# GiorgiaAuroraAdorni/gansformer-reproducibility-challenge

Measured on NVIDIA H100. Metric: images/sec @256^2 synth (GANsformer generator forward, K=16 latents, 12 attention layers, batch 32/GPU), higher is better.
Workload: dtype tf32 (fp32 storage; wgmma tf32 attention and stride-1 3x3 convolutions (own kernels), TF32 cuDNN up-convolutions; value_fp32_convs = the same with fp32 cuDNN convolutions)

## Files before the change

### gansformer-reproducibility-challenge_b200/csrc/gf_conv.cu

```cuda
#include <stdlib.h>
#include <string.h>
#include "gf_common.cuh"
#include "gf_tc_common.cuh"
#include "../../include/gf_ops.h"

namespace gf {
namespace cv {

using namespace tc;

constexpr int PH = 8, PW = 16;
constexpr int BK = 32;
constexpr int A_ROWS = (PH + 2) * PW;
constexpr int A_BYTES = A_ROWS * BK * 4;
constexpr int NUM_THREADS = 288;
constexpr int MAX_A = 3, MAX_W = 8;

struct Bars {
  uint64_t full_a[MAX_A], empty_a[MAX_A], full_w[MAX_W], empty_w[MAX_W];
};

struct Params {
  int B, H, W, Cin, Cout;
  int tiles_h, tiles_w, tiles_n;
  long long total_tiles;
  int na, nw;
  float alpha;
};

__device__ __forceinline__ void tma_load_4d(uint32_t dst, const CUtensorMap* map, uint32_t bar, int c0, int c1, int c2, int c3) {
  asm volatile(
      "cp.async.bulk.tensor.4d.shared::cluster.global.mbarrier::complete_tx::bytes [%0], [%1, {%3, %4, %5, %6}], [%2];"
      ::"r"(dst), "l"(map), "r"(bar), "r"(c0), "r"(c1), "r"(c2), "r"(c3)
      : "memory");
}

template <int BN>
__global__ void __launch_bounds__(NUM_THREADS, 1)
conv3x3_tc_kernel(const __grid_constant__ CUtensorMap tmX, const __grid_constant__ CUtensorMap tmW, float* __restrict__ y, const Params P) {
  constexpr int W_BYTES = BN * BK * 4;
  extern __shared__ __align__(1024) uint8_t smem_raw[];
  uint8_t* smem = smem_raw + ((1024u - (smem_u32(smem_raw) & 1023u)) & 1023u);
  const uint32_t s_a = smem_u32(smem);
  const uint32_t s_w = s_a + (uint32_t)P.na * A_BYTES;
  Bars* bars = reinterpret_cast<Bars*>(smem + (size_t)P.na * A_BYTES + (size_t)P.nw * W_BYTES);
  const int warp = __shfl_sync(0xffffffffu, (int)(threadIdx.x >> 5), 0);
  const int lane = threadIdx.x & 31;

  if (warp == 8 && lane == 0) {
    prefetch_tmap(&tmX); prefetch_tmap(&tmW);
    for (int i = 0; i < P.na; ++i) { mbar_init(smem_u32(&bars->full_a[i]), 1); mbar_init(smem_u32(&bars->empty_a[i]), 2); }
    for (int i = 0; i < P.nw; ++i) { mbar_init(smem_u32(&bars->full_w[i]), 1); mbar_init(smem_u32(&bars->empty_w[i]), 2); }
    fence_barrier_init();
  }
  __syncthreads();

  auto decode = [&](long long t, int& nt, int& pw, int& ph, int& b) {
    nt = (int)(t % P.tiles_n); t /= P.tiles_n;
    pw = (int)(t % P.tiles_w); t /= P.tiles_w;
    ph = (int)(t % P.tiles_h); b = (int)(t / P.tiles_h);
  };

  if (warp == 8) {
    if (lane == 0) {
      int sa = 0, sw = 0; uint32_t pa = 0, pw_ = 0;
      for (long long t = blockIdx.x; t < P.total_tiles; t += gridDim.x) {
        int nt, pw, ph, b;
        decode(t, nt, pw, ph, b);
        const int h0 = ph * PH, w0 = pw * PW, n0 = nt * BN;
        for (int c0 = 0; c0 < P.Cin; c0 += BK) {
          for (int dx = 0; dx < 3; ++dx) {
            mbar_wait(smem_u32(&bars->empty_a[sa]), pa ^ 1u);
            const uint32_t fa = smem_u32(&bars->full_a[sa]);
            mbar_expect_tx(fa, (uint32_t)A_BYTES);
            tma_load_4d(s_a + (uint32_t)sa * A_BYTES, &tmX, fa, c0, w0 + dx - 1, h0 - 1, b);
            if (++sa == P.na) { sa = 0; pa ^= 1u; }
            for (int dy = 0; dy < 3; ++dy) {
              mbar_wait(smem_u32(&bars->empty_w[sw]), pw_ ^ 1u);
              const uint32_t fw = smem_u32(&bars->full_w[sw]);
              mbar_expect_tx(fw, (uint32_t)W_BYTES);
              tma_load_2d(s_w + (uint32_t)sw * W_BYTES, &tmW, fw, c0, (dy * 3 + dx) * P.Cout + n0);
              if (++sw == P.nw) { sw = 0; pw_ ^= 1u; }
            }
          }
        }
      }
    }
    return;
  }

  const int wg = warp >> 2;
  const int gid = lane >> 2, qd = lane & 3;
  const int rA = wg * 64 + (warp & 3) * 16 + gid;
  const bool leader = (warp & 3) == 0 && lane == 0;
  int sa = 0, sw = 0; uint32_t pa = 0, pw_ = 0;
  for (long long t = blockIdx.x; t < P.total_tiles; t += gridDim.x) {
    int nt, pw, ph, b;
    decode(t, nt, pw, ph, b);
    float acc[BN / 2];
    int prev_w = -1, prev_a = -1;
#pragma unroll 1
    for (int c0 = 0; c0 < P.Cin; c0 += BK) {
#pragma unroll 1
      for (int dx = 0; dx < 3; ++dx) {
        mbar_wait(smem_u32(&bars->full_a[sa]), pa);
        const uint32_t a_view = s_a + (uint32_t)sa * A_BYTES + wg * 64 * 128;
#pragma unroll
        for (int dy = 0; dy < 3; ++dy) {
          mbar_wait(smem_u32(&bars->full_w[sw]), pw_);
          const uint64_t da = gmma_desc(a_view + dy * PW * 128, 1024, LAYOUT_SW128);
          const uint64_t db = gmma_desc(s_w + (uint32_t)sw * W_BYTES, 1024, LAYOUT_SW128);
          const uint32_t acc0 = (c0 | dx | dy) ? 1u : 0u;
          wgmma_fence();
#pragma unroll
          for (int kk = 0; kk < 4; ++kk) wgmma_ss<BN>(acc, da + kk * 2, db + kk * 2, (acc0 | kk) ? 1u : 0u);
          wgmma_commit();
          wgmma_wait<1>();
          if (prev_w >= 0) {
            named_bar_sync(1 + wg, 128);
            if (leader) {
              mbar_arrive(smem_u32(&bars->empty_w[prev_w]));
              if (prev_a >= 0) mbar_arrive(smem_u32(&bars->empty_a[prev_a]));
            }
          }
          prev_w = sw;
          prev_a = dy == 2 ? sa : -1;
          if (++sw == P.nw) { sw = 0; pw_ ^= 1u; }
        }
        if (++sa == P.na) { sa = 0; pa ^= 1u; }
      }
    }
    wgmma_wait<0>();
    fence_regs<BN / 2>(acc);
    named_bar_sync(1 + wg, 128);
    if (leader) {
      mbar_arrive(smem_u32(&bars->empty_w[prev_w]));
      mbar_arrive(smem_u32(&bars->empty_a[prev_a]));
    }
#pragma unroll
    for (int i = 0; i < 2; ++i) {
      const int r = rA + 8 * i;
      const int h = ph * PH + (r >> 4), w = pw * PW + (r & 15);
      float* yrow = y + (((size_t)b * P.H + h) * P.W + w) * P.Cout + nt * BN + 2 * qd;
#pragma unroll
      for (int j = 0; j < BN / 8; ++j)
        *reinterpret_cast<float2*>(yrow + 8 * j) = make_float2(acc[4 * j + 2 * i] * P.alpha, acc[4 * j + 2 * i + 1] * P.alpha);
    }
  }
}

constexpr int U_PC = 16, U_PR = 8;
constexpr int U_OC = U_PC - 2;
constexpr int U_BN = 64;
constexpr int U_A_BYTES = (U_PR + 1) * U_PC * BK * 4;
constexpr int U_W_BYTES = U_BN * BK * 4;
constexpr int U_CS = 68;
constexpr int U_MAX_A = 4, U_MAX_W = 10;

struct UBars {
  uint64_t full_a[U_MAX_A], empty_a[U_MAX_A], full_w[U_MAX_W], empty_w[U_MAX_W];
};

struct UParams {
  int B, H, W, Cin, Cout;
  int strips, steps, tiles_n;
  int total_units;
  int na, nw;
  float ag;
  const float* scale;
};

__device__ constexpr int U_TAP[9] = {0, 6, 3, 2, 1, 8, 7, 5, 4};
__device__ constexpr int U_PH[9] = {0, 0, 2, 0, 1, 0, 1, 2, 3};
__device__ constexpr int U_ROW0[9] = {1, 0, 0, 1, 1, 0, 0, 0, 0};
__device__ constexpr int U_FIRST[9] = {1, 0, 1, 0, 1, 0, 0, 0, 1};

__global__ void __launch_bounds__(NUM_THREADS, 1)
upconv_blur_tc_kernel(const __grid_constant__ CUtensorMap tmX, const __grid_constant__ CUtensorMap tmW, float* __restrict__ y, const UParams P) {
  extern __shared__ __align__(1024) uint8_t smem_raw[];
  uint8_t* smem = smem_raw + ((1024u - (smem_u32(smem_raw) & 1023u)) & 1023u);
  const uint32_t s_a = smem_u32(smem);
  const uint32_t s_w = s_a + (uint32_t)P.na * U_A_BYTES;
  float* carry = reinterpret_cast<float*>(smem + (size_t)P.na * U_A_BYTES + (size_t)P.nw * U_W_BYTES);
  float* stage = carry + 4 * 2 * U_PC * U_CS;
  UBars* bars = reinterpret_cast<UBars*>(stage + U_PR * U_PC * U_CS);
  const int warp = __shfl_sync(0xffffffffu, (int)(threadIdx.x >> 5), 0);
  const int lane = threadIdx.x & 31;

  if (warp == 8 && lane == 0) {
    prefetch_tmap(&tmX); prefetch_tmap(&tmW);
    for (int i = 0; i < P.na; ++i) { mbar_init(smem_u32(&bars->full_a[i]), 1); mbar_init(smem_u32(&bars->empty_a[i]), 2); }
    for (int i = 0; i < P.nw; ++i) { mbar_init(smem_u32(&bars->full_w[i]), 1); mbar_init(smem_u32(&bars->empty_w[i]), 2); }
    fence_barrier_init();
  }
  __syncthreads();

  auto decode = [&](int u, int& nt, int& st, int& b) {
    nt = u % P.tiles_n; u /= P.tiles_n;
    st = u % P.strips; b = u / P.strips;
  };

  if (warp == 8) {
    if (lane == 0) {
      int sa = 0, sw = 0; uint32_t pa = 0, pw_ = 0;
      for (int u = blockIdx.x; u < P.total_units; u += gridDim.x) {
        int nt, st, b;
        decode(u, nt, st, b);
        const int j0 = st * U_OC, n0 = nt * U_BN;
        for (int s = 0; s < P.steps; ++s) {
          for (int c0 = 0; c0 < P.Cin; c0 += BK) {
            for (int t = 0; t < 9; ++t) {
              if (t == 0 || t == 3) {
                mbar_wait(smem_u32(&bars->empty_a[sa]), pa ^ 1u);
                const uint32_t fa = smem_u32(&bars->full_a[sa]);
                mbar_expect_tx(fa, (uint32_t)U_A_BYTES);
                tma_load_4d(s_a + (uint32_t)sa * U_A_BYTES, &tmX, fa, c0, j0 - (t == 3), s * U_PR - 1, b);
                if (++sa == P.na) { sa = 0; pa ^= 1u; }
              }
              mbar_wait(smem_u32(&bars->empty_w[sw]), pw_ ^ 1u);
              const uint32_t fw = smem_u32(&bars->full_w[sw]);
              mbar_expect_tx(fw, (uint32_t)U_W_BYTES);
              tma_load_2d(s_w + (uint32_t)sw * U_W_BYTES, &tmW, fw, c0, U_TAP[t] * P.Cout + n0);
              if (++sw == P.nw) { sw = 0; pw_ ^= 1u; }
            }
          }
        }
      }
    }
    return;
  }

  const int wg = warp >> 2;
  const int gid = lane >> 2, qd = lane & 3;
  const bool leader = (warp & 3) == 0 && lane == 0;
  const int cp = lane & 7, cg = lane >> 3;
  int sa = 0, sw = 0; uint32_t pa = 0, pw_ = 0;
  for (int u = blockIdx.x; u < P.total_units; u += gridDim.x) {
    int nt, st, b;
    decode(u, nt, st, b);
    const int j0 = st * U_OC, n0 = nt * U_BN;
    for (int s = 0; s < P.steps; ++s) {
      float acc[4][U_BN / 2];
      int prev_w = -1, prev_a = -1;
      uint32_t a_view = 0;
#pragma unroll 1
      for (int c0 = 0; c0 < P.Cin; c0 += BK) {
#pragma unroll
        for (int t = 0; t < 9; ++t) {
          if (t == 0 || t == 3) {
            mbar_wait(smem_u32(&bars->full_a[sa]), pa);
            a_view = s_a + (uint32_t)sa * U_A_BYTES + wg * 4 * U_PC * 128;
          }
          mbar_wait(smem_u32(&bars->full_w[sw]), pw_);
          const uint64_t da = gmma_desc(a_view + U_ROW0[t] * U_PC * 128, 1024, LAYOUT_SW128);
          const uint64_t db = gmma_desc(s_w + (uint32_t)sw * U_W_BYTES, 1024, LAYOUT_SW128);
          const uint32_t acc0 = (c0 > 0 || !U_FIRST[t]) ? 1u : 0u;
          wgmma_fence();
#pragma unroll
          for (int kk = 0; kk < 4; ++kk) wgmma_ss<U_BN>(acc[U_PH[t]], da + kk * 2, db + kk * 2, (acc0 | kk) ? 1u : 0u);
          wgmma_commit();
          wgmma_wait<1>();
          if (prev_w >= 0) {
            named_bar_sync(1 + wg, 128);
            if (leader) {
              mbar_arrive(smem_u32(&bars->empty_w[prev_w]));
              if (prev_a >= 0) mbar_arrive(smem_u32(&bars->empty_a[prev_a]));
            }
          }
          prev_w = sw;
          prev_a = (t == 2 || t == 8) ? sa : -1;
          if (++sw == P.nw) { sw = 0; pw_ ^= 1u; }
          if (t == 2 || t == 8) { if (++sa == P.na) { sa = 0; pa ^= 1u; } }
        }
      }
      wgmma_wait<0>();
#pragma unroll
      for (int ph = 0; ph < 4; ++ph) fence_regs<U_BN / 2>(acc[ph]);
      named_bar_sync(1 + wg, 128);
      if (leader) {
        mbar_arrive(smem_u32(&bars->empty_w[prev_w]));
        mbar_arrive(smem_u32(&bars->empty_a[prev_a]));
      }

      const int io = s * U_PR - 2 + warp;
#pragma unroll
      for (int sl = 0; sl < U_BN / 16; ++sl) {
        float* my_row = stage + warp * U_PC * U_CS;
#pragma unroll
        for (int ph = 0; ph < 4; ++ph)
#pragma unroll
          for (int jj = 0; jj < 2; ++jj)
#pragma unroll
            for (int i = 0; i < 2; ++i)
              *reinterpret_cast<float2*>(my_row + (gid + 8 * i) * U_CS + ph * 16 + jj * 8 + 2 * qd) =
                  make_float2(acc[ph][4 * (2 * sl + jj) + 2 * i], acc[ph][4 * (2 * sl + jj) + 2 * i + 1]);
        named_bar_sync(3, 256);
        if (io >= 0 && io < P.H) {
          auto row = [&](int r) -> const float* {
            return (r < 2 ? carry + (sl * 2 + r) * U_PC * U_CS : stage + (r - 2) * U_PC * U_CS) + 2 * cp;
          };
          const int ch = n0 + sl * 16 + 2 * cp;
          const float2 d = __ldg(reinterpret_cast<const float2*>(P.scale + (size_t)b * P.Cout + ch));
          const float2 f = make_float2(P.ag * d.x, P.ag * d.y);
          const int Wo = 2 * P.W;
#pragma unroll 1
          for (int p = cg; p < U_OC && j0 + p < P.W; p += 4) {
            float* y0 = y + (((size_t)b * 2 * P.H + 2 * io) * Wo + 2 * (j0 + p)) * P.Cout + ch;
#pragma unroll 1
            for (int cb = 0; cb < 2; ++cb) {
              const int oA = cb ? 0 : 16, oB = cb ? U_CS + 16 : 0, oC = cb ? U_CS : U_CS + 16, oD = cb ? 2 * U_CS + 16 : U_CS;
              float2 e, o;
#pragma unroll
              for (int v = 0; v < 5; ++v) {
                const float* base = row(warp + v / 2) + ((v & 1) ? 0 : 32) + p * U_CS;
                const float2 A = *reinterpret_cast<const float2*>(base + oA), B_ = *reinterpret_cast<const float2*>(base + oB);
                const float2 C = *reinterpret_cast<const float2*>(base + oC), D = *reinterpret_cast<const float2*>(base + oD);
                float2 hv;
                hv.x = ((A.x + 3.f * B_.x) + 3.f * C.x) + D.x;
                hv.y = ((A.y + 3.f * B_.y) + 3.f * C.y) + D.y;
                if (v == 0) { e = hv; }
                else if (v == 1) { e.x += 3.f * hv.x; e.y += 3.f * hv.y; o = hv; }
                else if (v == 2) { e.x += 3.f * hv.x; e.y += 3.f * hv.y; o.x += 3.f * hv.x; o.y += 3.f * hv.y; }
                else if (v == 3) { e.x += hv.x; e.y += hv.y; o.x += 3.f * hv.x; o.y += 3.f * hv.y; }
                else { o.x += hv.x; o.y += hv.y; }
              }
              *reinterpret_cast<float2*>(y0 + cb * P.Cout) = make_float2(e.x * 0.015625f * f.x, e.y * 0.015625f * f.y);
              *reinterpret_cast<float2*>(y0 + (size_t)Wo * P.Cout + cb * P.Cout) = make_float2(o.x * 0.015625f * f.x, o.y * 0.015625f * f.y);
            }
          }
        }
        named_bar_sync(3, 256);
        if (warp >= U_PR - 2) {
          float* crow = carry + (sl * 2 + warp - (U_PR - 2)) * U_PC * U_CS;
#pragma unroll
          for (int ph = 0; ph < 4; ++ph)
#pragma unroll
            for (int jj = 0; jj < 2; ++jj)
#pragma unroll
              for (int i = 0; i < 2; ++i)
                *reinterpret_cast<float2*>(crow + (gid + 8 * i) * U_CS + ph * 16 + jj * 8 + 2 * qd) =
                    make_float2(acc[ph][4 * (2 * sl + jj) + 2 * i], acc[ph][4 * (2 * sl + jj) + 2 * i + 1]);
        }
      }
    }
  }
}

static int make_map_nhwc(CUtensorMap* m, const void* base, int B, int H, int W, int C, int box_c, int box_w, int box_h) {
  EncodeTiledFn enc = get_encode();
  if (!enc) { set_error("cuTensorMapEncodeTiled entry point not available"); return GF_ERR_CUDA; }
  cuuint64_t dims[4] = {(cuuint64_t)C, (cuuint64_t)W, (cuuint64_t)H, (cuuint64_t)B};
  cuuint64_t strides[3] = {(cuuint64_t)C * 4, (cuuint64_t)W * C * 4, (cuuint64_t)H * W * C * 4};
  cuuint32_t box[4] = {(cuuint32_t)box_c, (cuuint32_t)box_w, (cuuint32_t)box_h, 1};
  cuuint32_t estr[4] = {1, 1, 1, 1};
  CUresult r = enc(m, CU_TENSOR_MAP_DATA_TYPE_FLOAT32, 4, const_cast<void*>(base), dims, strides, box, estr, CU_TENSOR_MAP_INTERLEAVE_NONE,
                   CU_TENSOR_MAP_SWIZZLE_128B, CU_TENSOR_MAP_L2_PROMOTION_L2_128B, CU_TENSOR_MAP_FLOAT_OOB_FILL_NONE);
  if (r != CUDA_SUCCESS) { set_error("cuTensorMapEncodeTiled (NHWC 4-D) failed with CUresult %d (B=%d H=%d W=%d C=%d)", (int)r, B, H, W, C); return GF_ERR_CUDA; }
  return GF_OK;
}

template <int BN>
static int launch_bn(const float* x, const float* wt, float* y, int B, int H, int W, int Cin, int Cout, cudaStream_t st) {
  constexpr int W_BYTES = BN * BK * 4;
  CUtensorMap tmX, tmW;
  int rc;
  if ((rc = make_map_nhwc(&tmX, x, B, H, W, Cin, BK, PW, PH + 2))) return rc;
  if ((rc = make_map(&tmW, wt, (uint64_t)9 * Cout, (uint64_t)Cin, BN, BK, CU_TENSOR_MAP_SWIZZLE_128B))) return rc;
  Params P;
  P.B = B; P.H = H; P.W = W; P.Cin = Cin; P.Cout = Cout;
  P.tiles_h = H / PH; P.tiles_w = W / PW; P.tiles_n = Cout / BN;
  P.total_tiles = (long long)B * P.tiles_h * P.tiles_w * P.tiles_n;
  const int avail = device_smem_optin() - (int)sizeof(Bars) - 1024;
  P.na = MAX_A;
  P.nw = (avail - P.na * A_BYTES) / W_BYTES;
  if (P.nw > MAX_W) P.nw = MAX_W;
  if (P.nw < 2) { set_error("conv3x3: shared memory too small"); return GF_ERR_UNSUPPORTED; }
  P.alpha = 1.000352220f;
  const int smem_bytes = P.na * A_BYTES + P.nw * W_BYTES + (int)sizeof(Bars) + 1024;
  GF_CUDA_OK(cudaFuncSetAttribute(conv3x3_tc_kernel<BN>, cudaFuncAttributeMaxDynamicSharedMemorySize, smem_bytes));
  long long grid = device_sms();
  if (grid > P.total_tiles) grid = P.total_tiles;
  conv3x3_tc_kernel<BN><<<(unsigned)grid, NUM_THREADS, smem_bytes, st>>>(tmX, tmW, y, P);
  GF_LAUNCH_OK();
  return GF_OK;
}

static int launch(const float* x, const float* wt, float* y, int B, int H, int W, int Cin, int Cout, cudaStream_t st) {
  if (Cout % 256 == 0) return launch_bn<256>(x, wt, y, B, H, W, Cin, Cout, st);
  if (Cout % 128 == 0) return launch_bn<128>(x, wt, y, B, H, W, Cin, Cout, st);
  return launch_bn<64>(x, wt, y, B, H, W, Cin, Cout, st);
}

static int launch_upconv(const float* x, const float* wt, const float* scale, float* y, int B, int H, int W, int Cin, int Cout,
                         float gain, cudaStream_t st) {
  CUtensorMap tmX, tmW;
  int rc;
  if ((rc = make_map_nhwc(&tmX, x, B, H, W, Cin, BK, U_PC, U_PR + 1))) return rc;
  if ((rc = make_map(&tmW, wt, (uint64_t)9 * Cout, (uint64_t)Cin, U_BN, BK, CU_TENSOR_MAP_SWIZZLE_128B))) return rc;
  UParams P;
  P.B = B; P.H = H; P.W = W; P.Cin = Cin; P.Cout = Cout;
  P.strips = (W + U_OC - 1) / U_OC;
  P.steps = (H + 2 + U_PR - 1) / U_PR;
  P.tiles_n = Cout / U_BN;
  const long long units = (long long)B * P.strips * P.tiles_n;
  if (units > (1ll << 30)) { set_error("upconv3x3_blur: too many work units (%lld)", units); return GF_ERR_UNSUPPORTED; }
  P.total_units = (int)units;
  P.ag = 1.000352220f * gain;
  P.scale = scale;
  const int fixed = 8 * U_PC * U_CS * 4 + U_PR * U_PC * U_CS * 4 + (int)sizeof(UBars) + 1024;
  P.na = U_MAX_A;
  P.nw = (device_smem_optin() - fixed - P.na * U_A_BYTES) / U_W_BYTES;
  if (P.nw > U_MAX_W) P.nw = U_MAX_W;
  if (P.nw < 3) { set_error("upconv3x3_blur: shared memory too small"); return GF_ERR_UNSUPPORTED; }
  const int smem_bytes = fixed + P.na * U_A_BYTES + P.nw * U_W_BYTES;
  GF_CUDA_OK(cudaFuncSetAttribute(upconv_blur_tc_kernel, cudaFuncAttributeMaxDynamicSharedMemorySize, smem_bytes));
  long long grid = device_sms();
  if (grid > P.total_units) grid = P.total_units;
  upconv_blur_tc_kernel<<<(unsigned)grid, NUM_THREADS, smem_bytes, st>>>(tmX, tmW, y, P);
  GF_LAUNCH_OK();
  return GF_OK;
}

__global__ void pack_weights_kernel(const float* __restrict__ w, float* __restrict__ wt, int Cout, int Cin, float scale) {
  const size_t total = (size_t)9 * Cout * Cin;
  for (size_t i = blockIdx.x * (size_t)blockDim.x + threadIdx.x; i < total; i += (size_t)gridDim.x * blockDim.x) {
    const int ci = (int)(i % Cin);
    const int o = (int)((i / Cin) % Cout);
    const int tap = (int)(i / ((size_t)Cin * Cout));
    wt[i] = round_tf32_rn(w[((size_t)o * Cin + ci) * 9 + tap] * scale);
  }
}

}
}

using namespace gf;

extern "C" int gf_conv3x3_pack_weights(const float* w, float* wt, int Cout, int Cin, float scale, void* stream) {
  if (!w || !wt || Cout <= 0 || Cin <= 0) { set_error("gf_conv3x3_pack_weights: bad arguments"); return GF_ERR_INVALID; }
  const size_t total = (size_t)9 * Cout * Cin;
  size_t blocks = (total + 255) / 256;
  if (blocks > (size_t)num_sms() * 16) blocks = (size_t)num_sms() * 16;
  cv::pack_weights_kernel<<<(unsigned)blocks, 256, 0, (cudaStream_t)stream>>>(w, wt, Cout, Cin, scale);
  GF_LAUNCH_OK();
  return GF_OK;
}

extern "C" int gf_conv3x3_nhwc_tf32(const float* x, const float* wt, float* y, int B, int H, int W, int Cin, int Cout, void* stream) {
  if (!x || !wt || !y) { set_error("gf_conv3x3_nhwc_tf32: null pointer"); return GF_ERR_INVALID; }
  if (B <= 0 || H <= 0 || W <= 0 || H % cv::PH || W % cv::PW || Cin % cv::BK || Cout % 64 || Cin <= 0 || Cout <= 0) {
    set_error("gf_conv3x3_nhwc_tf32: needs positive sizes, H %% 8 == 0, W %% 16 == 0, Cin %% 32 == 0, Cout %% 64 == 0 (got B=%d H=%d W=%d Cin=%d Cout=%d)", B, H, W, Cin, Cout);
    return GF_ERR_UNSUPPORTED;
  }
  if (((uintptr_t)x & 15) || ((uintptr_t)wt & 15) || ((uintptr_t)y & 15)) { set_error("gf_conv3x3_nhwc_tf32: pointers must be 16-byte aligned"); return GF_ERR_INVALID; }
  int rc;
  if ((rc = check_device())) return rc;
  return cv::launch(x, wt, y, B, H, W, Cin, Cout, (cudaStream_t)stream);
}

extern "C" int gf_upconv3x3_blur_nhwc_tf32(const float* x, const float* wt, const float* scale, float* y, int B, int H, int W, int Cin,
                                           int Cout, float gain, void* stream) {
  if (!x || !wt || !scale || !y) { set_error("gf_upconv3x3_blur_nhwc_tf32: null pointer"); return GF_ERR_INVALID; }
  if (B <= 0 || H <= 0 || W <= 0 || Cin <= 0 || Cout <= 0 || Cin % cv::BK || Cout % cv::U_BN) {
    set_error("gf_upconv3x3_blur_nhwc_tf32: needs positive sizes, Cin %% 32 == 0, Cout %% 64 == 0 (got B=%d H=%d W=%d Cin=%d Cout=%d)", B, H, W, Cin, Cout);
    return GF_ERR_UNSUPPORTED;
  }
  if (((uintptr_t)x & 15) || ((uintptr_t)wt & 15) || ((uintptr_t)y & 15) || ((uintptr_t)scale & 15)) {
    set_error("gf_upconv3x3_blur_nhwc_tf32: pointers must be 16-byte aligned"); return GF_ERR_INVALID;
  }
  int rc;
  if ((rc = check_device())) return rc;
  return cv::launch_upconv(x, wt, scale, y, B, H, W, Cin, Cout, gain, (cudaStream_t)stream);
}
```

### gansformer-reproducibility-challenge_b200/networks.py

```python
from __future__ import annotations

import math
import os
from typing import List, Optional

import numpy as np
import torch
import torch.nn.functional as F
from torch import nn

from .attention import BipartiteAttention, _Plan, prologue_batch, tc_eligible
from . import ops
from ._state import weights_epoch, bump_weights_epoch
from .ops import fir_filter

SQRT2 = math.sqrt(2.0)


def _inference(*params) -> bool:
    return not (torch.is_grad_enabled() and any(p.requires_grad for p in params))


UPCONV_FUSED_MIN_RES = 256

CACHE_BYPASS = False


def _cached(module: nn.Module, key: str, params, fn):
    if CACHE_BYPASS:
        with torch.no_grad():
            return fn()
    ver = (weights_epoch(),) + tuple((p.data_ptr(), p._version, str(p.device), p.dtype) for p in params)
    store = module.__dict__.setdefault("_icache", {})
    ent = store.get(key)
    if ent is None or ent[0] != ver:
        with torch.no_grad():
            ent = (ver, fn())
        store[key] = ent
    return ent[1]


RUNTIME_KEYS = ("_icache", "_graphs", "_side_stream", "_copy_stream")


def drop_runtime_state(module: nn.Module) -> nn.Module:
    for m in module.modules():
        for key in [k for k in m.__dict__ if k in RUNTIME_KEYS or (isinstance(k, tuple) and k and k[0] == "_staging")]:
            del m.__dict__[key]
        if isinstance(m, BipartiteAttention):
            m._plan = _Plan()
    return module


def nf(res: int, fmap_base: int = 16384, fmap_max: int = 512) -> int:
    return int(min(fmap_base // (2 ** (int(math.log2(res)) - 1)), fmap_max))


def modulated_conv2d(x: torch.Tensor, weight: torch.Tensor, styles: torch.Tensor, *, demodulate: bool = True,
                     up: int = 1, f: Optional[torch.Tensor] = None, w_eff: Optional[torch.Tensor] = None,
                     wsq: Optional[torch.Tensor] = None, prescaled: bool = False, defer_demod: bool = False,
                     d: Optional[torch.Tensor] = None, phases=None, wt_packed: Optional[torch.Tensor] = None):
    O, I, kh, kw = weight.shape
    if w_eff is None:
        w_eff = weight * (1.0 / math.sqrt(I * kh * kw))
        if up != 1:
            w_eff = w_eff.transpose(0, 1)
    if demodulate and d is None:
        if wsq is None:
            wsq = (weight * (1.0 / math.sqrt(I * kh * kw))).square().sum(dim=[2, 3])
        d = ops.demod_coef(styles, wsq)
    if not prescaled:
        x = ops.chan_scale(x, styles)
    if up == 1:
        if wt_packed is not None:
            x = ops.conv3x3_native(x, wt_packed)
        else:
            x = F.conv2d(x, w_eff, padding=kh // 2)
        if defer_demod:
            return x, d
        if d is not None:
            x = ops.chan_scale(x, d)
    elif wt_packed is not None and d is not None and ops._use_cuda(x, d):
        x = ops.upconv_blur_native(x, wt_packed, scale=d, gain=4.0)
    elif phases is not None and ops._use_cuda(x, d) and O % 4 == 0 and not os.environ.get("GF_NO_PHASES"):
        x = ops.upconv_blur_phases(x, phases, scale=d, gain=4.0)
    else:
        x = F.conv_transpose2d(x, w_eff, stride=2)
        x = ops.blur_up(x, f, scale=d, gain=4.0)
    return x


class FullyConnected(nn.Module):
    def __init__(self, in_features: int, out_features: int, bias_init: float = 0.0, lr_mul: float = 1.0, act: str = "linear"):
        super().__init__()
        self.weight = nn.Parameter(torch.randn(out_features, in_features) / lr_mul)
        self.bias = nn.Parameter(torch.full((out_features,), float(bias_init)))
        self.wgain = lr_mul / math.sqrt(in_features)
        self.bgain = lr_mul
        self.act = act

    def effective(self):
        g = SQRT2 if self.act == "lrelu" else 1.0
        return (self.weight * (self.wgain * g)).t().contiguous(), self.bias * (self.bgain * g)

    def forward(self, x):
        if _inference(self.weight, self.bias):
            wt, b = _cached(self, "eff", (self.weight, self.bias), self.effective)
            y = torch.addmm(b, x.reshape(-1, x.shape[-1]), wt).reshape(*x.shape[:-1], wt.shape[1])
            return F.leaky_relu(y, 0.2) if self.act == "lrelu" else y
        x = F.linear(x, self.weight * self.wgain, self.bias * self.bgain)
        return F.leaky_relu(x, 0.2) * SQRT2 if self.act == "lrelu" else x


class MappingNetwork(nn.Module):

    def __init__(self, latent_dim: int, components_num: int, num_layers: int = 8, lr_mul: float = 0.01, ltnt2ltnt: bool = False,
                 integration: str = "mul", norm: Optional[str] = "layer", exact_fp32: bool = False):
        super().__init__()
        self.latent_dim, self.components_num = latent_dim, components_num
        self.local = nn.ModuleList([FullyConnected(latent_dim, latent_dim, lr_mul=lr_mul, act="lrelu") for _ in range(num_layers)])
        self.glob = nn.ModuleList([FullyConnected(latent_dim, latent_dim, lr_mul=lr_mul, act="lrelu") for _ in range(num_layers)])
        self.register_buffer("w_avg", torch.zeros(2, latent_dim))
        self.self_att = None
        if ltnt2ltnt and components_num > 1:
            self.self_att = nn.ModuleList([BipartiteAttention(latent_dim, latent_dim, components_num, pos_dim=latent_dim, use_pos=False,
                                                              integration=integration, norm=norm, exact_fp32=exact_fp32)
                                           for _ in range(num_layers)])

    def forward(self, z: torch.Tensor, truncation_psi: float = 1.0) -> torch.Tensor:
        k = self.components_num
        if z.dim() != 3 or z.shape[1] != k + 1 or z.shape[2] != self.latent_dim:
            raise ValueError(f"z must be [B, {k + 1}, {self.latent_dim}], got {tuple(z.shape)}")
        params = [t for fc in list(self.local) + list(self.glob) for t in (fc.weight, fc.bias)]
        if (self.self_att is None and z.is_cuda and z.dtype == torch.float32 and _inference(*params) and self.latent_dim <= 128
                and len(self.local) * self.latent_dim ** 2 * 8 <= 200 * 1024 and not os.environ.get("GF_NO_MAPPING_KERNEL")):
            def stack():
                wl, bl = zip(*[fc.effective() for fc in self.local])
                wg, bg = zip(*[fc.effective() for fc in self.glob])
                return (torch.stack([torch.stack(wl), torch.stack(wg)]).contiguous(), torch.stack([torch.stack(bl), torch.stack(bg)]).contiguous())
            w_eff, b_eff = _cached(self, "stack", params, stack)
            return ops.mapping_fwd(z, w_eff, b_eff, self.w_avg, float(truncation_psi), k)
        z = z * torch.rsqrt(z.square().mean(dim=2, keepdim=True) + 1e-8)
        loc, glo = z[:, :k], z[:, k:]
        for i, fc in enumerate(self.local):
            loc = fc(loc)
            if self.self_att is not None:
                loc = loc.contiguous()
                loc, _, _ = self.self_att[i](loc.reshape(loc.shape[0], k, 1, self.latent_dim), loc)
                loc = loc.reshape(-1, k, self.latent_dim)
        for fc in self.glob:
            glo = fc(glo)
        if truncation_psi != 1.0:
            loc = self.w_avg[0].lerp(loc, truncation_psi)
            glo = self.w_avg[1].lerp(glo, truncation_psi)
        return torch.cat([loc, glo], dim=1)


class SynthesisLayer(nn.Module):

    def __init__(self, in_ch: int, out_ch: int, w_dim: int, resolution: int, up: bool, components_num: int,
                 use_attention: bool, attn_kwargs: dict):
        super().__init__()
        self.resolution, self.up = resolution, up
        self.affine = FullyConnected(w_dim, in_ch, bias_init=1.0)
        self.weight = nn.Parameter(torch.randn(out_ch, in_ch, 3, 3))
        self.bias = nn.Parameter(torch.zeros(out_ch))
        self.register_buffer("noise_const", torch.randn(resolution, resolution))
        self.noise_strength = nn.Parameter(torch.zeros([]))
        self.register_buffer("fir", fir_filter())
        self.attention = BipartiteAttention(out_ch, w_dim, components_num, **attn_kwargs) if use_attention else None

    def _conv_weights(self):
        O, I, kh, kw = self.weight.shape
        w = self.weight * (1.0 / math.sqrt(I * kh * kw))
        wsq = w.square().sum(dim=[2, 3])
        phases = ops.upconv_phase_weights(w) if self.up else None
        packed = None
        if w.is_cuda and kh == 3 and I % 32 == 0 and O % 64 == 0 and (not self.up or self.resolution >= UPCONV_FUSED_MIN_RES):
            packed = ops.conv3x3_pack(w)
        if self.up:
            w = w.transpose(0, 1)
        return w.contiguous(memory_format=torch.channels_last), wsq.contiguous(), phases, packed

    def fusable(self, x) -> bool:
        a = self.attention
        return (a is not None and x.is_cuda and a.norm in ("layer", None, "none")
                and _inference(self.weight, self.bias, self.noise_strength, *a.parameters()))

    def forward(self, x, w_glob, y, noise_mode="const", centroids=None, return_att=False, styles=None,
                prescaled=False, post_scale=None, prepared=None, rgb=None, centroids_init=None, demod=None):
        if styles is None:
            styles = self.affine(w_glob)
        w_eff = wsq = phases = packed = None
        if _inference(self.weight) and x.is_cuda:
            w_eff, wsq, phases, packed = _cached(self, "conv", (self.weight,), self._conv_weights)
            if packed is not None and not (torch.backends.cudnn.allow_tf32 and x.dtype == torch.float32
                                           and (self.up or (x.shape[2] % 8 == 0 and x.shape[3] % 16 == 0
                                                            and not os.environ.get("GF_CUDNN_CONV")))):
                packed = None
        fused = self.fusable(x)
        in_scale = None
        if prepared is not None and not fused:
            raise RuntimeError("internal: prepared prologue for a layer that does not take the fused path")
        if fused and not self.up:
            x, in_scale = modulated_conv2d(x, self.weight, styles, up=1, f=self.fir, w_eff=w_eff, wsq=wsq,
                                           prescaled=prescaled, defer_demod=True, d=prepared[1] if prepared is not None else demod,
                                           wt_packed=packed)
        else:
            x = modulated_conv2d(x, self.weight, styles, up=2 if self.up else 1, f=self.fir, w_eff=w_eff, wsq=wsq,
                                 prescaled=prescaled, phases=phases, wt_packed=packed, d=demod)
        if noise_mode == "const":
            noise = self.noise_const
        elif noise_mode == "random":
            noise = torch.randn(x.shape[0], 1, self.resolution, self.resolution, device=x.device, dtype=x.dtype)
        else:
            noise = None
        att = None
        if self.attention is not None:
            xl = x.permute(0, 2, 3, 1)
            if not xl.is_contiguous():
                xl = xl.contiguous()
            if fused:
                post = dict(bias=self.bias, noise=noise, strength=self.noise_strength, act="lrelu", gain=SQRT2,
                            in_scale=in_scale, post_scale=post_scale)
                if rgb is not None:
                    post.update(rgb)
                post.update(self.attention.dropout_postop(x.device))
                if prepared is not None and prepared[0] is not None:
                    torch.cuda.current_stream(x.device).wait_event(prepared[0])
                xo, att, centroids = self.attention(xl, y, centroids=centroids, return_att=return_att, postop=post,
                                                    stage="token" if prepared is not None else "all",
                                                    need_centroids=self.attention.iterative,
                                                    centroids_init=centroids_init)
                return xo.permute(0, 3, 1, 2), att, centroids
            xo, att, centroids = self.attention(xl, y, centroids=centroids, return_att=return_att, centroids_init=centroids_init)
            x = xo.permute(0, 3, 1, 2)
        x = ops.bias_act(x, self.bias, "lrelu", noise=noise, strength=self.noise_strength)
        if post_scale is not None:
            x = ops.chan_scale(x, post_scale)
        return x, att, centroids


class ToRGB(nn.Module):
    def __init__(self, in_ch: int, w_dim: int, img_channels: int = 3):
        super().__init__()
        self.affine = FullyConnected(w_dim, in_ch, bias_init=1.0)
        self.weight = nn.Parameter(torch.randn(img_channels, in_ch, 1, 1))
        self.bias = nn.Parameter(torch.zeros(img_channels))

    def forward(self, x, w_glob, styles=None, next_styles=None):
        if styles is None:
            styles = self.affine(w_glob)
        return ops.torgb(x, self.weight, styles, self.bias, next_styles=next_styles)


class SynthesisNetwork(nn.Module):

    def __init__(self, resolution: int, latent_dim: int, components_num: int, fmap_base: int = 16384, fmap_max: int = 512,
                 g_start_res: int = 8, g_end_res: Optional[int] = None, transformer: bool = True, attn_kwargs: Optional[dict] = None):
        super().__init__()
        assert resolution >= 4 and resolution & (resolution - 1) == 0
        self.resolution, self.components_num = resolution, components_num
        g_end_res = resolution if g_end_res is None else g_end_res
        self.block_resolutions = [2 ** i for i in range(2, int(math.log2(resolution)) + 1)]
        attn_kwargs = dict(attn_kwargs or {})
        self.const = nn.Parameter(torch.randn(nf(4, fmap_base, fmap_max), 4, 4))
        self.layers = nn.ModuleList()
        self.torgbs = nn.ModuleList()
        self.layer_res: List[int] = []
        self.iterative = bool(attn_kwargs.get("iterative", False)) and bool(attn_kwargs.get("kmeans", False))
        for res in self.block_resolutions:
            out_ch = nf(res, fmap_base, fmap_max)
            use_att = transformer and components_num > 0 and g_start_res <= res <= g_end_res
            if res > 4:
                in_ch = nf(res // 2, fmap_base, fmap_max)
                self.layers.append(SynthesisLayer(in_ch, out_ch, latent_dim, res, True, components_num, use_att, attn_kwargs))
                self.layer_res.append(res)
            self.layers.append(SynthesisLayer(out_ch, out_ch, latent_dim, res, False, components_num, use_att, attn_kwargs))
            self.layer_res.append(res)
            self.torgbs.append(ToRGB(out_ch, latent_dim))
        self.register_buffer("fir", fir_filter())
        self.num_attention_layers = sum(1 for l in self.layers if l.attention is not None)

    def forward(self, ws: torch.Tensor, noise_mode: str = "const", return_att: bool = False, return_features: bool = False):
        k = self.components_num
        B = ws.shape[0]
        y = ws[:, :k].contiguous()
        w_glob = ws[:, k]
        x = self.const[None].expand(B, -1, -1, -1).contiguous(memory_format=torch.channels_last)
        mods = list(self.layers) + list(self.torgbs)
        aff = [m.affine for m in mods]
        aff_params = [t for a in aff for t in (a.weight, a.bias)]
        styles_all = [None] * len(mods)
        if _inference(*aff_params):
            def cat_affines():
                ws_, bs_ = zip(*[a.effective() for a in aff])
                return torch.cat(ws_, dim=1).contiguous(), torch.cat(bs_)
            wt_cat, b_cat = _cached(self, "affines", aff_params, cat_affines)
            styles_all = torch.addmm(b_cat, w_glob, wt_cat).split([a.weight.shape[0] for a in aff], dim=1)
        prepared = [None] * len(self.layers)
        demods = [None] * len(self.layers)
        if x.is_cuda and styles_all[0] is not None and _inference(*[l.weight for l in self.layers]):
            demods = ops.demod_coef_batch([(styles_all[li_], _cached(l, "conv", (l.weight,), l._conv_weights)[1])
                                           for li_, l in enumerate(self.layers)])
        if x.is_cuda and styles_all[0] is not None and not os.environ.get("GF_NO_BATCH_PROLOGUE"):
            items = []
            for li_, layer in enumerate(self.layers):
                if not layer.fusable(x):
                    continue
                d_ = None
                if not layer.up:
                    d_ = demods[li_]
                    if d_ is None:
                        _, wsq_, _, _ = _cached(layer, "conv", (layer.weight,), layer._conv_weights)
                        d_ = ops.demod_coef(styles_all[li_], wsq_)
                C_ = layer.weight.shape[0]
                items.append((layer.attention, y, (B, layer.resolution, layer.resolution, C_), d_))
                prepared[li_] = (None, d_)
            prologue_batch(items)
        img = None
        atts = []
        feats = []
        li = 0
        block_prescaled = False
        cen_prev = None
        for bi, res in enumerate(self.block_resolutions):
            nl = 1 if res == 4 else 2
            prescaled = block_prescaled
            nxt = styles_all[li + nl] if (li + nl < len(self.layers) and styles_all[li + nl] is not None and x.is_cuda and not return_features
                                          and not os.environ.get("GF_NO_TORGB_FUSE")) else None
            rgb = None
            for j in range(nl):
                layer = self.layers[li]
                cen_init = None
                if self.iterative and layer.attention is not None and cen_prev is not None and cen_prev.shape[2] == layer.weight.shape[0] \
                        and _inference(*layer.attention.parameters()):
                    cen_init = cen_prev
                post_scale = None
                if j == 0 and nl == 2 and styles_all[li + 1] is not None and layer.fusable(x) and not return_features:
                    post_scale = styles_all[li + 1]
                rgb_args = None
                if j == nl - 1 and layer.fusable(x) and not return_features and not os.environ.get("GF_NO_TORGB_EPILOGUE"):
                    C_ = layer.weight.shape[0]
                    tg = self.torgbs[bi]
                    if (C_ <= 256 or (k <= 16 and not os.environ.get("GF_TORGB_EPILOGUE_C256"))) and _inference(tg.weight, tg.bias) \
                            and tc_eligible(layer.attention, (B, res, res, C_), k):
                        st_rgb = styles_all[len(self.layers) + bi]
                        rgb_w = (tg.weight.reshape(1, 3, C_) * st_rgb[:, None, :] * (1.0 / math.sqrt(C_))).contiguous()
                        rgb = torch.empty((B, 3, res, res), device=x.device, dtype=torch.float32)
                        rgb_args = dict(rgb_w=rgb_w, rgb_bias=tg.bias, rgb_out=rgb)
                        post_scale = nxt
                x, att, cen_out = layer(x, w_glob, y, noise_mode=noise_mode, return_att=return_att, styles=styles_all[li],
                                        prescaled=prescaled, post_scale=post_scale, prepared=prepared[li], rgb=rgb_args,
                                        centroids_init=cen_init, demod=demods[li])
                if layer.attention is not None:
                    cen_prev = cen_out if self.iterative else None
                prescaled = post_scale is not None
                li += 1
                if att is not None:
                    atts.append(att)
                if return_features and layer.attention is not None:
                    feats.append(x)
            if rgb is not None:
                block_prescaled = nxt is not None
            else:
                rgb = self.torgbs[bi](x, w_glob, styles=styles_all[len(self.layers) + bi], next_styles=nxt)
                block_prescaled = nxt is not None
                if block_prescaled:
                    rgb, x = rgb
            img = rgb if img is None else ops.upsample2x(img, self.fir, add=rgb)
        out = (img,) + ((atts,) if return_att else ()) + ((feats,) if return_features else ())
        return out[0] if len(out) == 1 else out


class Generator(nn.Module):

    def __init__(self, resolution: int = 256, components_num: int = 16, latent_size: int = 512, latent_dim: Optional[int] = None,
                 transformer: bool = True, g_start_res: int = 8, g_end_res: Optional[int] = None, kmeans: bool = False,
                 kmeans_iters: int = 1, iterative: bool = False, integration: str = "mul", norm: Optional[str] = "layer",
                 use_pos: bool = True, pos_dim: Optional[int] = None, num_heads: int = 1, mapping_layers: int = 8,
                 fmap_base: int = 16384, fmap_max: int = 512, exact_fp32: bool = False, ltnt2ltnt: bool = False, g_img2ltnt: bool = False,
                 att_dp: float = 0.0):
        super().__init__()
        self.latent_dim = latent_dim if latent_dim is not None else max(latent_size // max(components_num, 1), 1)
        self.components_num, self.resolution = components_num, resolution
        attn_kwargs = dict(pos_dim=pos_dim, num_heads=num_heads, integration=integration, norm=norm, kmeans=kmeans,
                           kmeans_iters=kmeans_iters, use_pos=use_pos, exact_fp32=exact_fp32, iterative=iterative,
                           img2ltnt=bool(g_img2ltnt and kmeans), att_dp=att_dp)
        self.mapping = MappingNetwork(self.latent_dim, components_num, num_layers=mapping_layers, ltnt2ltnt=ltnt2ltnt,
                                      integration=integration, norm=norm, exact_fp32=exact_fp32)
        self.synthesis = SynthesisNetwork(resolution, self.latent_dim, components_num, fmap_base=fmap_base, fmap_max=fmap_max,
                                          g_start_res=g_start_res, g_end_res=g_end_res, transformer=transformer,
                                          attn_kwargs=attn_kwargs)

    def forward(self, z: torch.Tensor, c=None, truncation_psi: float = 1.0, noise_mode: str = "const", return_att: bool = False,
                return_features: bool = False):
        ws = self.mapping(z, truncation_psi=truncation_psi)
        return self.synthesis(ws, noise_mode=noise_mode, return_att=return_att, return_features=return_features)

    def __deepcopy__(self, memo):
        import copy as _copy
        new = self.__class__.__new__(self.__class__)
        memo[id(self)] = new
        for k_, v_ in self.__dict__.items():
            if k_ in RUNTIME_KEYS or isinstance(k_, tuple):
                continue
            new.__dict__[k_] = _copy.deepcopy(v_, memo)
        return drop_runtime_state(new)

    def load_state_dict(self, *args, **kwargs):
        res = super().load_state_dict(*args, **kwargs)
        bump_weights_epoch()
        drop_runtime_state(self)
        return res

    @torch.no_grad()
    def graphed(self, batch_size: int, truncation_psi: float = 1.0, noise_mode: str = "const"):
        key = (batch_size, float(truncation_psi), noise_mode, weights_epoch(), bool(torch.backends.cudnn.allow_tf32), bool(os.environ.get("GF_CUDNN_CONV")),
               tuple((p.data_ptr(), p._version) for p in self.parameters()))
        cache = self.__dict__.setdefault("_graphs", {})
        if key in cache:
            return cache[key]
        cache.clear()
        dev = next(self.parameters()).device
        if dev.type != "cuda":
            raise RuntimeError("CUDA graphs need the generator on a CUDA device")
        static_z = torch.zeros(batch_size, self.components_num + 1, self.latent_dim, device=dev)
        side = torch.cuda.Stream(device=dev)
        side.wait_stream(torch.cuda.current_stream(dev))
        with torch.cuda.stream(side):
            for _ in range(3):
                self(static_z, truncation_psi=truncation_psi, noise_mode=noise_mode)
        torch.cuda.current_stream(dev).wait_stream(side)
        graph = torch.cuda.CUDAGraph()
        with torch.cuda.graph(graph):
            static_img = self(static_z, truncation_psi=truncation_psi, noise_mode=noise_mode)

        def replay(z: torch.Tensor) -> torch.Tensor:
            static_z.copy_(z, non_blocking=True)
            graph.replay()
            return static_img

        cache[key] = replay
        return replay

    @torch.no_grad()
    def run(self, latents, labels=None, truncation_psi: float = 1.0, randomize_noise: bool = False, minibatch_size: int = 32,
            cuda_graph: bool = False, out: Optional[torch.Tensor] = None):
        dev = next(self.parameters()).device
        lat = torch.as_tensor(np.asarray(latents) if not torch.is_tensor(latents) else latents, dtype=torch.float32)
        n = lat.shape[0]
        noise_mode = "random" if randomize_noise else "const"
        res = out if out is not None else torch.empty((n, 3, self.resolution, self.resolution), dtype=torch.float32)
        if dev.type != "cuda":
            for i in range(0, n, minibatch_size):
                z = lat[i:i + minibatch_size].to(dev)
                res[i:i + z.shape[0]].copy_(self(z, truncation_psi=truncation_psi, noise_mode=noise_mode))
            return res
        main = torch.cuda.current_stream(dev)
        copy_stream = self.__dict__.get("_copy_stream")
        if copy_stream is None or copy_stream.device != dev:
            copy_stream = self.__dict__["_copy_stream"] = torch.cuda.Stream(device=dev)
        skey = ("_staging", minibatch_size)
        staging = self.__dict__.get(skey)
        if staging is None or staging[0].device != dev:
            staging = self.__dict__[skey] = [torch.empty((minibatch_size, 3, self.resolution, self.resolution), device=dev) for _ in range(2)]
        d2h_done = [None, None]
        for idx, i in enumerate(range(0, n, minibatch_size)):
            z = lat[i:i + minibatch_size].to(dev, non_blocking=True)
            m = z.shape[0]
            if cuda_graph and m == minibatch_size:
                img = self.graphed(minibatch_size, truncation_psi, noise_mode)(z)
            else:
                img = self(z, truncation_psi=truncation_psi, noise_mode=noise_mode)
            sidx = idx & 1
            if d2h_done[sidx] is not None:
                main.wait_event(d2h_done[sidx])
            staging[sidx][:m].copy_(img)
            ready = torch.cuda.Event()
            ready.record(main)
            with torch.cuda.stream(copy_stream):
# ... 8 lines not shown
```

Measured before the change: 1627.

## Group upconv phase taps into wide wgmma and add register-rebalanced warpgroups

Restructures the fused upconv+blur kernel so the nine per-tap weight loads become four grouped TMA loads. Each group issues a single N=128 or N=64 wgmma that covers two output phases sharing an A view, and all nine tap weights for a K-slice stay resident in shared memory. It adds a third warpgroup so setmaxnreg can move registers from the producer to the consumers, and computes both horizontal blur outputs in one pass to reuse shared-memory loads. It also turns on the fused path at resolution 8. The trade-offs are a fixed and larger weight footprint with fewer pipeline stages, and 128 extra idle threads.

```diff
diff --git a/gansformer-reproducibility-challenge_b200/csrc/gf_conv.cu b/gansformer-reproducibility-challenge_b200/csrc/gf_conv.cu
--- a/gansformer-reproducibility-challenge_b200/csrc/gf_conv.cu
+++ b/gansformer-reproducibility-challenge_b200/csrc/gf_conv.cu
@@ -154,34 +154,39 @@
 constexpr int U_BN = 64;
 constexpr int U_A_BYTES = (U_PR + 1) * U_PC * BK * 4;
 constexpr int U_W_BYTES = U_BN * BK * 4;
+constexpr int U_WS_BYTES = 9 * U_W_BYTES;
 constexpr int U_CS = 68;
-constexpr int U_MAX_A = 4, U_MAX_W = 10;
+constexpr int U_NA = 4;
+constexpr int U_THREADS = 384;
 
 struct UBars {
-  uint64_t full_a[U_MAX_A], empty_a[U_MAX_A], full_w[U_MAX_W], empty_w[U_MAX_W];
+  uint64_t full_a[U_NA], empty_a[U_NA], full_w[4], empty_w[4];
 };
 
 struct UParams {
   int B, H, W, Cin, Cout;
   int strips, steps, tiles_n;
   int total_units;
-  int na, nw;
   float ag;
   const float* scale;
 };
 
-__device__ constexpr int U_TAP[9] = {0, 6, 3, 2, 1, 8, 7, 5, 4};
-__device__ constexpr int U_PH[9] = {0, 0, 2, 0, 1, 0, 1, 2, 3};
-__device__ constexpr int U_ROW0[9] = {1, 0, 0, 1, 1, 0, 0, 0, 0};
-__device__ constexpr int U_FIRST[9] = {1, 0, 1, 0, 1, 0, 0, 0, 1};
-
-__global__ void __launch_bounds__(NUM_THREADS, 1)
+__device__ constexpr int U_GTAPS[4] = {4, 2, 2, 1};
+__device__ constexpr int U_GNX[4] = {2, 2, 1, 1};
+__device__ constexpr int U_GTAP[4][4] = {{8, 7, 5, 4}, {2, 1, 0, 0}, {6, 3, 0, 0}, {0, 0, 0, 0}};
+__device__ constexpr int U_GOFF[4] = {0, 4, 6, 8};
+__device__ constexpr int U_GROW[4] = {0, 1, 0, 1};
+
+__device__ __forceinline__ void setmaxnreg_dec40() { asm volatile("setmaxnreg.dec.sync.aligned.u32 40;"); }
+__device__ __forceinline__ void setmaxnreg_inc232() { asm volatile("setmaxnreg.inc.sync.aligned.u32 232;"); }
+
+__global__ void __launch_bounds__(U_THREADS, 1)
 upconv_blur_tc_kernel(const __grid_constant__ CUtensorMap tmX, const __grid_constant__ CUtensorMap tmW, float* __restrict__ y, const UParams P) {
   extern __shared__ __align__(1024) uint8_t smem_raw[];
   uint8_t* smem = smem_raw + ((1024u - (smem_u32(smem_raw) & 1023u)) & 1023u);
   const uint32_t s_a = smem_u32(smem);
-  const uint32_t s_w = s_a + (uint32_t)P.na * U_A_BYTES;
-  float* carry = reinterpret_cast<float*>(smem + (size_t)P.na * U_A_BYTES + (size_t)P.nw * U_W_BYTES);
+  const uint32_t s_w = s_a + (uint32_t)U_NA * U_A_BYTES;
+  float* carry = reinterpret_cast<float*>(smem + (size_t)U_NA * U_A_BYTES + U_WS_BYTES);
   float* stage = carry + 4 * 2 * U_PC * U_CS;
   UBars* bars = reinterpret_cast<UBars*>(stage + U_PR * U_PC * U_CS);
   const int warp = __shfl_sync(0xffffffffu, (int)(threadIdx.x >> 5), 0);
@@ -189,8 +194,8 @@
 
   if (warp == 8 && lane == 0) {
     prefetch_tmap(&tmX); prefetch_tmap(&tmW);
-    for (int i = 0; i < P.na; ++i) { mbar_init(smem_u32(&bars->full_a[i]), 1); mbar_init(smem_u32(&bars->empty_a[i]), 2); }
-    for (int i = 0; i < P.nw; ++i) { mbar_init(smem_u32(&bars->full_w[i]), 1); mbar_init(smem_u32(&bars->empty_w[i]), 2); }
+    for (int i = 0; i < U_NA; ++i) { mbar_init(smem_u32(&bars->full_a[i]), 1); mbar_init(smem_u32(&bars->empty_a[i]), 2); }
+    for (int i = 0; i < 4; ++i) { mbar_init(smem_u32(&bars->full_w[i]), 1); mbar_init(smem_u32(&bars->empty_w[i]), 2); }
     fence_barrier_init();
   }
   __syncthreads();
@@ -200,29 +205,31 @@
     st = u % P.strips; b = u / P.strips;
   };
 
-  if (warp == 8) {
-    if (lane == 0) {
-      int sa = 0, sw = 0; uint32_t pa = 0, pw_ = 0;
+  if (warp >= 8) {
+    setmaxnreg_dec40();
+    if (warp == 8 && lane == 0) {
+      int sa = 0; uint32_t pa = 0, pw_ = 0;
       for (int u = blockIdx.x; u < P.total_units; u += gridDim.x) {
         int nt, st, b;
         decode(u, nt, st, b);
         const int j0 = st * U_OC, n0 = nt * U_BN;
         for (int s = 0; s < P.steps; ++s) {
           for (int c0 = 0; c0 < P.Cin; c0 += BK) {
-            for (int t = 0; t < 9; ++t) {
-              if (t == 0 || t == 3) {
+            for (int g = 0; g < 4; ++g) {
+              if (g == 0 || g == 2) {
                 mbar_wait(smem_u32(&bars->empty_a[sa]), pa ^ 1u);
                 const uint32_t fa = smem_u32(&bars->full_a[sa]);
                 mbar_expect_tx(fa, (uint32_t)U_A_BYTES);
-                tma_load_4d(s_a + (uint32_t)sa * U_A_BYTES, &tmX, fa, c0, j0 - (t == 3), s * U_PR - 1, b);
-                if (++sa == P.na) { sa = 0; pa ^= 1u; }
+                tma_load_4d(s_a + (uint32_t)sa * U_A_BYTES, &tmX, fa, c0, j0 - (g == 0), s * U_PR - 1, b);
+                if (++sa == U_NA) { sa = 0; pa ^= 1u; }
               }
-              mbar_wait(smem_u32(&bars->empty_w[sw]), pw_ ^ 1u);
-              const uint32_t fw = smem_u32(&bars->full_w[sw]);
-              mbar_expect_tx(fw, (uint32_t)U_W_BYTES);
-              tma_load_2d(s_w + (uint32_t)sw * U_W_BYTES, &tmW, fw, c0, U_TAP[t] * P.Cout + n0);
-              if (++sw == P.nw) { sw = 0; pw_ ^= 1u; }
+              mbar_wait(smem_u32(&bars->empty_w[g]), pw_ ^ 1u);
+              const uint32_t fw = smem_u32(&bars->full_w[g]);
+              mbar_expect_tx(fw, (uint32_t)(U_GTAPS[g] * U_W_BYTES));
+              for (int k = 0; k < U_GTAPS[g]; ++k)
+                tma_load_2d(s_w + (uint32_t)(U_GOFF[g] + k) * U_W_BYTES, &tmW, fw, c0, U_GTAP[g][k] * P.Cout + n0);
             }
+            pw_ ^= 1u;
           }
         }
       }
@@ -230,55 +237,63 @@
     return;
   }
 
+  setmaxnreg_inc232();
   const int wg = warp >> 2;
   const int gid = lane >> 2, qd = lane & 3;
   const bool leader = (warp & 3) == 0 && lane == 0;
   const int cp = lane & 7, cg = lane >> 3;
-  int sa = 0, sw = 0; uint32_t pa = 0, pw_ = 0;
+  int sa = 0; uint32_t pa = 0, pw_ = 0;
   for (int u = blockIdx.x; u < P.total_units; u += gridDim.x) {
     int nt, st, b;
     decode(u, nt, st, b);
     const int j0 = st * U_OC, n0 = nt * U_BN;
     for (int s = 0; s < P.steps; ++s) {
-      float acc[4][U_BN / 2];
-      int prev_w = -1, prev_a = -1;
+      float accx[U_BN], accy[U_BN];
+      int prev_a = -1;
       uint32_t a_view = 0;
 #pragma unroll 1
       for (int c0 = 0; c0 < P.Cin; c0 += BK) {
 #pragma unroll
-        for (int t = 0; t < 9; ++t) {
-          if (t == 0 || t == 3) {
+        for (int g = 0; g < 4; ++g) {
+          if (g == 0 || g == 2) {
             mbar_wait(smem_u32(&bars->full_a[sa]), pa);
             a_view = s_a + (uint32_t)sa * U_A_BYTES + wg * 4 * U_PC * 128;
           }
-          mbar_wait(smem_u32(&bars->full_w[sw]), pw_);
-          const uint64_t da = gmma_desc(a_view + U_ROW0[t] * U_PC * 128, 1024, LAYOUT_SW128);
-          const uint64_t db = gmma_desc(s_w + (uint32_t)sw * U_W_BYTES, 1024, LAYOUT_SW128);
-          const uint32_t acc0 = (c0 > 0 || !U_FIRST[t]) ? 1u : 0u;
+          mbar_wait(smem_u32(&bars->full_w[g]), pw_);
+          const uint64_t da = gmma_desc(a_view + U_GROW[g] * U_PC * 128, 1024, LAYOUT_SW128);
+          const uint64_t db = gmma_desc(s_w + (uint32_t)U_GOFF[g] * U_W_BYTES, 1024, LAYOUT_SW128);
+          const uint64_t dby = db + (uint64_t)(U_GNX[g] * U_W_BYTES >> 4);
+          const int ny = U_GTAPS[g] - U_GNX[g];
+          const uint32_t acc0 = (c0 > 0 || g > 0) ? 1u : 0u;
           wgmma_fence();
 #pragma unroll
-          for (int kk = 0; kk < 4; ++kk) wgmma_ss<U_BN>(acc[U_PH[t]], da + kk * 2, db + kk * 2, (acc0 | kk) ? 1u : 0u);
+          for (int kk = 0; kk < 4; ++kk) {
+            const uint32_t ac = (acc0 | kk) ? 1u : 0u;
+            if (U_GNX[g] == 2) wgmma_ss<128>(accx, da + kk * 2, db + kk * 2, ac);
+            else wgmma_ss<64>(accx, da + kk * 2, db + kk * 2, ac);
+            if (ny == 2) wgmma_ss<128>(accy, da + kk * 2, dby + kk * 2, ac);
+            else if (ny == 1) wgmma_ss<64>(accy, da + kk * 2, dby + kk * 2, ac);
+          }
           wgmma_commit();
           wgmma_wait<1>();
-          if (prev_w >= 0) {
+          if (c0 > 0 || g > 0) {
             named_bar_sync(1 + wg, 128);
             if (leader) {
-              mbar_arrive(smem_u32(&bars->empty_w[prev_w]));
+              mbar_arrive(smem_u32(&bars->empty_w[(g + 3) & 3]));
               if (prev_a >= 0) mbar_arrive(smem_u32(&bars->empty_a[prev_a]));
             }
           }
-          prev_w = sw;
-          prev_a = (t == 2 || t == 8) ? sa : -1;
-          if (++sw == P.nw) { sw = 0; pw_ ^= 1u; }
-          if (t == 2 || t == 8) { if (++sa == P.na) { sa = 0; pa ^= 1u; } }
-        }
+          prev_a = (g == 1 || g == 3) ? sa : -1;
+          if (g == 1 || g == 3) { if (++sa == U_NA) { sa = 0; pa ^= 1u; } }
+        }
+        pw_ ^= 1u;
       }
       wgmma_wait<0>();
-#pragma unroll
-      for (int ph = 0; ph < 4; ++ph) fence_regs<U_BN / 2>(acc[ph]);
+      fence_regs<U_BN>(accx);
+      fence_regs<U_BN>(accy);
       named_bar_sync(1 + wg, 128);
       if (leader) {
-        mbar_arrive(smem_u32(&bars->empty_w[prev_w]));
+        mbar_arrive(smem_u32(&bars->empty_w[3]));
         mbar_arrive(smem_u32(&bars->empty_a[prev_a]));
       }
 
@@ -293,7 +308,7 @@
 #pragma unroll
             for (int i = 0; i < 2; ++i)
               *reinterpret_cast<float2*>(my_row + (gid + 8 * i) * U_CS + ph * 16 + jj * 8 + 2 * qd) =
-                  make_float2(acc[ph][4 * (2 * sl + jj) + 2 * i], acc[ph][4 * (2 * sl + jj) + 2 * i + 1]);
+                  make_float2((ph < 2 ? accx : accy)[32 * (ph & 1) + 4 * (2 * sl + jj) + 2 * i], (ph < 2 ? accx : accy)[32 * (ph & 1) + 4 * (2 * sl + jj) + 2 * i + 1]);
         named_bar_sync(3, 256);
         if (io >= 0 && io < P.H) {
           auto row = [&](int r) -> const float* {
@@ -306,27 +321,37 @@
 #pragma unroll 1
           for (int p = cg; p < U_OC && j0 + p < P.W; p += 4) {
             float* y0 = y + (((size_t)b * 2 * P.H + 2 * io) * Wo + 2 * (j0 + p)) * P.Cout + ch;
-#pragma unroll 1
-            for (int cb = 0; cb < 2; ++cb) {
-              const int oA = cb ? 0 : 16, oB = cb ? U_CS + 16 : 0, oC = cb ? U_CS : U_CS + 16, oD = cb ? 2 * U_CS + 16 : U_CS;
-              float2 e, o;
-#pragma unroll
-              for (int v = 0; v < 5; ++v) {
-                const float* base = row(warp + v / 2) + ((v & 1) ? 0 : 32) + p * U_CS;
-                const float2 A = *reinterpret_cast<const float2*>(base + oA), B_ = *reinterpret_cast<const float2*>(base + oB);
-                const float2 C = *reinterpret_cast<const float2*>(base + oC), D = *reinterpret_cast<const float2*>(base + oD);
-                float2 hv;
-                hv.x = ((A.x + 3.f * B_.x) + 3.f * C.x) + D.x;
-                hv.y = ((A.y + 3.f * B_.y) + 3.f * C.y) + D.y;
-                if (v == 0) { e = hv; }
-                else if (v == 1) { e.x += 3.f * hv.x; e.y += 3.f * hv.y; o = hv; }
-                else if (v == 2) { e.x += 3.f * hv.x; e.y += 3.f * hv.y; o.x += 3.f * hv.x; o.y += 3.f * hv.y; }
-                else if (v == 3) { e.x += hv.x; e.y += hv.y; o.x += 3.f * hv.x; o.y += 3.f * hv.y; }
-                else { o.x += hv.x; o.y += hv.y; }
+            float2 e0, o0, e1, o1;
+#pragma unroll
+            for (int v = 0; v < 5; ++v) {
+              const float* base = row(warp + v / 2) + ((v & 1) ? 0 : 32) + p * U_CS;
+              const float2 E0 = *reinterpret_cast<const float2*>(base), O0 = *reinterpret_cast<const float2*>(base + 16);
+              const float2 E1 = *reinterpret_cast<const float2*>(base + U_CS), O1 = *reinterpret_cast<const float2*>(base + U_CS + 16);
+              const float2 O2 = *reinterpret_cast<const float2*>(base + 2 * U_CS + 16);
+              float2 h0, h1;
+              h0.x = ((O0.x + 3.f * E0.x) + 3.f * O1.x) + E1.x;
+              h0.y = ((O0.y + 3.f * E0.y) + 3.f * O1.y) + E1.y;
+              h1.x = ((E0.x + 3.f * O1.x) + 3.f * E1.x) + O2.x;
+              h1.y = ((E0.y + 3.f * O1.y) + 3.f * E1.y) + O2.y;
+              if (v == 0) { e0 = h0; e1 = h1; }
+              else if (v == 1) {
+                e0.x += 3.f * h0.x; e0.y += 3.f * h0.y; o0 = h0;
+                e1.x += 3.f * h1.x; e1.y += 3.f * h1.y; o1 = h1;
+              } else if (v == 2) {
+                e0.x += 3.f * h0.x; e0.y += 3.f * h0.y; o0.x += 3.f * h0.x; o0.y += 3.f * h0.y;
+                e1.x += 3.f * h1.x; e1.y += 3.f * h1.y; o1.x += 3.f * h1.x; o1.y += 3.f * h1.y;
+              } else if (v == 3) {
+                e0.x += h0.x; e0.y += h0.y; o0.x += 3.f * h0.x; o0.y += 3.f * h0.y;
+                e1.x += h1.x; e1.y += h1.y; o1.x += 3.f * h1.x; o1.y += 3.f * h1.y;
+              } else {
+                o0.x += h0.x; o0.y += h0.y;
+                o1.x += h1.x; o1.y += h1.y;
               }
-              *reinterpret_cast<float2*>(y0 + cb * P.Cout) = make_float2(e.x * 0.015625f * f.x, e.y * 0.015625f * f.y);
-              *reinterpret_cast<float2*>(y0 + (size_t)Wo * P.Cout + cb * P.Cout) = make_float2(o.x * 0.015625f * f.x, o.y * 0.015625f * f.y);
             }
+            *reinterpret_cast<float2*>(y0) = make_float2(e0.x * 0.015625f * f.x, e0.y * 0.015625f * f.y);
+            *reinterpret_cast<float2*>(y0 + P.Cout) = make_float2(e1.x * 0.015625f * f.x, e1.y * 0.015625f * f.y);
+            *reinterpret_cast<float2*>(y0 + (size_t)Wo * P.Cout) = make_float2(o0.x * 0.015625f * f.x, o0.y * 0.015625f * f.y);
+            *reinterpret_cast<float2*>(y0 + (size_t)Wo * P.Cout + P.Cout) = make_float2(o1.x * 0.015625f * f.x, o1.y * 0.015625f * f.y);
           }
         }
         named_bar_sync(3, 256);
@@ -339,7 +364,7 @@
 #pragma unroll
               for (int i = 0; i < 2; ++i)
                 *reinterpret_cast<float2*>(crow + (gid + 8 * i) * U_CS + ph * 16 + jj * 8 + 2 * qd) =
-                    make_float2(acc[ph][4 * (2 * sl + jj) + 2 * i], acc[ph][4 * (2 * sl + jj) + 2 * i + 1]);
+                    make_float2((ph < 2 ? accx : accy)[32 * (ph & 1) + 4 * (2 * sl + jj) + 2 * i], (ph < 2 ? accx : accy)[32 * (ph & 1) + 4 * (2 * sl + jj) + 2 * i + 1]);
         }
       }
     }
@@ -407,16 +432,12 @@
   P.total_units = (int)units;
   P.ag = 1.000352220f * gain;
   P.scale = scale;
-  const int fixed = 8 * U_PC * U_CS * 4 + U_PR * U_PC * U_CS * 4 + (int)sizeof(UBars) + 1024;
-  P.na = U_MAX_A;
-  P.nw = (device_smem_optin() - fixed - P.na * U_A_BYTES) / U_W_BYTES;
-  if (P.nw > U_MAX_W) P.nw = U_MAX_W;
-  if (P.nw < 3) { set_error("upconv3x3_blur: shared memory too small"); return GF_ERR_UNSUPPORTED; }
-  const int smem_bytes = fixed + P.na * U_A_BYTES + P.nw * U_W_BYTES;
+  const int smem_bytes = U_NA * U_A_BYTES + U_WS_BYTES + 8 * U_PC * U_CS * 4 + U_PR * U_PC * U_CS * 4 + (int)sizeof(UBars) + 1024;
+  if (smem_bytes > device_smem_optin()) { set_error("upconv3x3_blur: shared memory too small"); return GF_ERR_UNSUPPORTED; }
   GF_CUDA_OK(cudaFuncSetAttribute(upconv_blur_tc_kernel, cudaFuncAttributeMaxDynamicSharedMemorySize, smem_bytes));
   long long grid = device_sms();
   if (grid > P.total_units) grid = P.total_units;
-  upconv_blur_tc_kernel<<<(unsigned)grid, NUM_THREADS, smem_bytes, st>>>(tmX, tmW, y, P);
+  upconv_blur_tc_kernel<<<(unsigned)grid, U_THREADS, smem_bytes, st>>>(tmX, tmW, y, P);
   GF_LAUNCH_OK();
   return GF_OK;
 }
diff --git a/gansformer-reproducibility-challenge_b200/networks.py b/gansformer-reproducibility-challenge_b200/networks.py
--- a/gansformer-reproducibility-challenge_b200/networks.py
+++ b/gansformer-reproducibility-challenge_b200/networks.py
@@ -21,7 +21,8 @@
     return not (torch.is_grad_enabled() and any(p.requires_grad for p in params))
 
 
-UPCONV_FUSED_MIN_RES = 256
+def upconv_fused(res: int) -> bool:
+    return res == 8 or res >= 256
 
 CACHE_BYPASS = False
 
@@ -176,7 +177,7 @@
         wsq = w.square().sum(dim=[2, 3])
         phases = ops.upconv_phase_weights(w) if self.up else None
         packed = None
-        if w.is_cuda and kh == 3 and I % 32 == 0 and O % 64 == 0 and (not self.up or self.resolution >= UPCONV_FUSED_MIN_RES):
+        if w.is_cuda and kh == 3 and I % 32 == 0 and O % 64 == 0 and (not self.up or upconv_fused(self.resolution)):
             packed = ops.conv3x3_pack(w)
         if self.up:
             w = w.transpose(0, 1)
```

Result: faster. 1710 (median of 6 runs) (+5.1%).
